# argumentcomputer/multi-stark

Hardware: AMD Instinct MI355X
Metric: prove_trace_rows_per_sec (higher is better)
Workload: dtype u64; 1 GPU; U32-add + byte-table lookup (benches/multi_stark.rs), 2^20 additions per proof, bench_config(): log_blowup 2, 100 queries, 10+10 PoW bits, GoldilocksBlake3Config; witness (traces + claims, 64-bit words) in pinned host memory at step start: upload, from_stage_1 on the device and read-back inside the timed region; the library narrows byte-valued traces on host threads INSIDE the step before they cro; rows_per_proof=1048832, proof_bytes=1100053, parallelism=single GPU

## Files before the change

multi-stark_amd/csrc/prover.hip:

```cpp
#include <algorithm>
#include <chrono>
#include <cstdio>
#include <cstdlib>

#include <sys/resource.h>
#include <unistd.h>

#include <atomic>
#include <condition_variable>
#include <functional>
#include <mutex>
#include <thread>

#include "host.h"
#include "ingest.h"
#include "lookup_params.h"
#include "open_plan.h"
#include "quotient_params.h"

namespace msamd {

namespace {
void load_block(const uint8_t* p, size_t len, u32 w[16]) {
  uint8_t buf[64];
  memset(buf, 0, 64);
  if (len) memcpy(buf, p, len);
  for (int i = 0; i < 16; i++)
    w[i] = (u32)buf[4 * i] | ((u32)buf[4 * i + 1] << 8) | ((u32)buf[4 * i + 2] << 16) | ((u32)buf[4 * i + 3] << 24);
}
void subtree_cv(const uint8_t* in, size_t len, u64 chunk_index, u32 root_flag, u32 out[8]) {
  if (len <= 1024) {
    b3_iv(out);
    size_t nblocks = len == 0 ? 1 : (len + 63) / 64;
    for (size_t b = 0; b < nblocks; b++) {
      size_t off = b * 64, bl = len - off < 64 ? len - off : 64;
      u32 m[16];
      load_block(in + off, bl, m);
      u32 flags = (b == 0 ? B3_CHUNK_START : 0) | (b == nblocks - 1 ? (B3_CHUNK_END | root_flag) : 0);
      b3_compress(out, m, chunk_index, (u32)bl, flags);
    }
    return;
  }
  size_t full = (len - 1) / 1024, lc = 1;
  while (lc * 2 <= full) lc *= 2;
  u32 m[16];
  subtree_cv(in, lc * 1024, chunk_index, 0, m);
  subtree_cv(in + lc * 1024, len - lc * 1024, chunk_index + lc, 0, m + 8);
  b3_iv(out);
  b3_compress(out, m, 0, 64, B3_PARENT | root_flag);
}
double now_ms() {
  return std::chrono::duration<double, std::milli>(std::chrono::steady_clock::now().time_since_epoch()).count();
}

struct HostProbes {
  bool on = false;
  double t0 = 0;
  long faults0 = 0;
  struct Mark {
    const char* what;
    double t;
    long faults;
  };
  std::vector<Mark> marks;
  static long faults_now() {
    struct rusage ru;
    return getrusage(RUSAGE_THREAD, &ru) == 0 ? ru.ru_minflt : 0;
  }
  void start() {
    on = getenv("MSAMD_TRACE_HOST") != nullptr;
    marks.clear();
    t0 = now_ms();
    if (on) faults0 = faults_now();
  }
  void mark(const char* what) {
    if (on) marks.push_back(Mark{what, now_ms(), faults_now()});
  }
  void print() const {
    if (!on) return;
    double prev = t0;
    long pf = faults0;
    for (auto& m : marks) {
      fprintf(stderr, "[msamd]   %-34s at %8.1f us (+%7.1f)  page faults +%ld\n", m.what, 1e3 * (m.t - t0), 1e3 * (m.t - prev), m.faults - pf);
      prev = m.t;
      pf = m.faults;
    }
  }
};
thread_local HostProbes g_probes;
}

void blake3_host(const uint8_t* in, size_t len, uint8_t out[32]) {
  u32 cv[8];
  subtree_cv(in, len, 0, B3_ROOT, cv);
  for (int i = 0; i < 8; i++)
    for (int k = 0; k < 4; k++) out[4 * i + k] = (uint8_t)(cv[i] >> (8 * k));
}

uint8_t Challenger::sample_byte() {
  if (output.empty()) {
    uint8_t d[32];
    blake3_host(input.data(), input.size(), d);
    input.assign(d, d + 32);
    output.assign(d, d + 32);
  }
  uint8_t b = output.back();
  output.pop_back();
  return b;
}
u64 Challenger::sample_u64() {
  u64 v = 0;
  for (int k = 0; k < 8; k++) v |= (u64)sample_byte() << (8 * k);
  return v;
}
u64 Challenger::sample_base() {
  for (;;) {
    u64 v = sample_u64();
    if (v < GL_P) return v;
  }
}
E2 Challenger::sample_ext() {
  u64 a = sample_base();
  u64 b = sample_base();
  return e2(a, b);
}
size_t Challenger::sample_bits(unsigned bits) { return (size_t)(sample_u64() & ((u64(1) << bits) - 1)); }

u64 Challenger::grind(unsigned bits) {
  if (bits == 0) return 0;
  std::vector<uint8_t> buf(input);
  size_t base = buf.size();
  buf.resize(base + 8);
  const u64 mask = (u64(1) << bits) - 1;
  for (u64 w = 0;; w++) {
    for (int k = 0; k < 8; k++) buf[base + k] = (uint8_t)(w >> (8 * k));
    uint8_t d[32];
    blake3_host(buf.data(), buf.size(), d);
    u64 v = 0;
    for (int k = 0; k < 8; k++) v |= (u64)d[31 - k] << (8 * k);
    if ((v & mask) == 0) {
      observe(w);
      size_t s = sample_bits(bits);
      if (s != 0) throw std::runtime_error("grind: internal inconsistency");
      return w;
    }
  }
}

namespace {
struct Reader {
  const uint8_t* p;
  size_t n, off = 0;
  u64 word() {
    if (off + 8 > n) throw std::runtime_error("system blob truncated");
    u64 v;
    memcpy(&v, p + off, 8);
    off += 8;
    return v;
  }
};
const u64 BLOB_MAGIC = 0x31305359534D0000ULL;
}

void commit_matrices(Ctx& ctx, std::vector<DMat>&& ldes, unsigned cap_height, PcsData& out) {
  out.ldes = std::move(ldes);
  out.tree = DTree();
  out.tree.cap_height = cap_height;
  for (auto& m : out.ldes) {
    out.tree.mat_d.push_back(m.d());
    out.tree.mat_h.push_back(m.h);
    out.tree.mat_w.push_back(m.w);
  }
  merkle_build(ctx, out.tree);
}

static DMat lde_of_host_matrix(Ctx& ctx, const u64* rowmajor_dev, size_t h, size_t w, unsigned lb) {
  unsigned logn = log2_strict(h);
  DBuf<u64> ev(ctx, h * w);
  transpose_in(ctx, rowmajor_dev, ev.p, h, w, true);
  DMat lde;
  lde.h = h << lb;
  lde.w = w;
  lde.buf = DBuf<u64>(ctx, lde.h * w);
  coset_lde(ctx, ev.p, lde.d(), logn, lb, w);
  return lde;
}

std::unique_ptr<HSystem> system_from_blob(Ctx& ctx, const uint8_t* blob, size_t len) {
  HIP_CHECK(hipSetDevice(ctx.device));
  Reader rd{blob, len};
  if (rd.word() != BLOB_MAGIC) throw std::runtime_error("bad system blob magic");
  std::unique_ptr<HSystem> sys(new HSystem());
  sys->ctx = &ctx;
  Params& p = sys->params;
  p.log_blowup = rd.word();
  p.cap_height = rd.word();
  p.log_final_poly_len = rd.word();
  p.max_log_arity = rd.word();
  p.num_queries = rd.word();
  p.commit_pow_bits = rd.word();
  p.query_pow_bits = rd.word();
  if (p.max_log_arity < 1 || p.max_log_arity > FRI_MAX_LOG_ARITY) throw std::runtime_error("max_log_arity must be 1 .. 6 (a FRI row is hashed as one BLAKE3 chunk)");
  if (p.log_blowup < 1 || p.log_blowup > 8) throw std::runtime_error("log_blowup out of range");
  if (p.commit_pow_bits > 40 || p.query_pow_bits > 40) throw std::runtime_error("proof-of-work bits out of range");
  {
    const char* tag = "multi-stark/v0";
    sys->seed.assign(tag, tag + 14);
    const u64 ps[7] = {p.log_blowup, p.cap_height, p.log_final_poly_len, p.max_log_arity, p.num_queries, p.commit_pow_bits,
                       p.query_pow_bits};
    for (u64 x : ps)
      for (int k = 0; k < 8; k++) sys->seed.push_back((uint8_t)(x >> (8 * k)));
  }
  const size_t D = 2;
  size_t nc = rd.word();
  std::vector<DMat> pre_ldes;
  for (size_t ci = 0; ci < nc; ci++) {
    sys->circuits.emplace_back();
    HCircuit& c = sys->circuits.back();
    c.main_width = rd.word();
    c.pre_width = rd.word();
    c.pre_height = rd.word();
    size_t nn = rd.word(), nz = rd.word(), nl = rd.word();
    c.num_lookups = nl;
    c.stage2_width = std::max<size_t>(nl, 1) * D;
    c.nodes.resize(nn);
    c.degrees.resize(nn);
    for (size_t i = 0; i < nn; i++) {
      u64 w0 = rd.word();
      PNode& nd = c.nodes[i];
      nd.kind = (uint32_t)(w0 & 0xff);
      nd.source = (uint32_t)((w0 >> 8) & 0xff);
      nd.offset = (uint32_t)((w0 >> 16) & 0xff);
// ... 216 lines not shown
void check_claims(size_t n_claims, const u64* offsets, const u64* data) {
  if (offsets[0] != 0) throw std::runtime_error("claim offsets must start at 0");
  for (size_t i = 0; i < n_claims; i++)
    if (offsets[i + 1] < offsets[i]) throw std::runtime_error("claim offsets must be non-decreasing");
  for (size_t i = 0, tot = (size_t)offsets[n_claims]; i < tot; i++)
    if (data[i] >= GL_P) throw std::runtime_error("non-canonical claim value");
}
}

std::unique_ptr<HWitness> witness_create_device(HSystem& sys, const ms_dev_matrix* traces, size_t n_claims, const u64* claim_offsets,
                                                const u64* claim_data, bool claims_on_device, void* producer_stream) {
  Ctx& ctx = *sys.ctx;
  HIP_CHECK(hipSetDevice(ctx.device));
  const size_t C = sys.circuits.size();
  if (!traces) throw std::runtime_error("ms_witness_create_device: null trace list");
  if (!claim_offsets) throw std::runtime_error("ms_witness_create_device: null claim offsets");
  std::vector<IngestView> views(C);
  std::vector<size_t> heights(C, 0);
  for (size_t ci = 0; ci < C; ci++) {
    const HCircuit& c = sys.circuits[ci];
    const size_t h = (size_t)traces[ci].height;
    heights[ci] = h;
    if (h == 0) continue;
    if (h & (h - 1)) throw std::runtime_error("trace height must be a power of two");
    if (log2_strict(h) > NTT_MAX_LOG || log2_strict(h) + sys.params.log_blowup > TW_LOG)
      throw std::runtime_error("trace height exceeds the supported maximum");
    if (c.pre_width && h != c.pre_height) throw std::runtime_error("main trace height must equal preprocessed trace height");
    views[ci] = ingest_check(ctx, traces[ci], ci, c.main_width, 8);
  }
  size_t tot = 0;
  if (claims_on_device) {
    ingest_check_device_range(ctx, claim_offsets, (n_claims + 1) * 8, 8, "device claim offsets");
  } else {
    tot = (size_t)claim_offsets[n_claims];
    if (tot && !claim_data) throw std::runtime_error("ms_witness_create_device: null claim data");
    check_claims(n_claims, claim_offsets, claim_data);
  }
  ingest_wait_for_producer(ctx, producer_stream);
  try {
    DBuf<u64> bad(ctx, C);
    if (C) HIP_CHECK(hipMemsetAsync(bad.p, 0xFF, C * 8, ctx.stream));
    std::vector<DBuf<u64>> dtr(C);
    for (size_t ci = 0; ci < C; ci++) {
      if (!heights[ci]) continue;
      dtr[ci] = DBuf<u64>(ctx, heights[ci] * views[ci].w);
      ingest_goldilocks(ctx, views[ci], dtr[ci].p, bad.p + ci);
    }
    DBuf<u64> d_offs(ctx, n_claims + 1), d_data;
    u64 tot_dev = 0;
    if (claims_on_device) {
      HIP_CHECK(hipMemcpyAsync(d_offs.p, claim_offsets, (n_claims + 1) * 8, hipMemcpyDeviceToDevice, ctx.stream));
      ctx.d2h_queue(&tot_dev, claim_offsets + n_claims, 8);
    } else {
      d_data = DBuf<u64>(ctx, std::max<size_t>(tot, 1));
      ctx.h2d(d_offs.p, claim_offsets, (n_claims + 1) * 8);
      if (tot) ctx.h2d(d_data.p, claim_data, tot * 8);
    }
    std::vector<u64> bad_h(C, ~u64(0));
    ctx.d2h(bad_h.data(), bad.p, C * 8);
    for (size_t ci = 0; ci < C; ci++)
      if (heights[ci] && bad_h[ci] != ~u64(0)) throw std::runtime_error(ingest_offender_text(ci, bad_h[ci], views[ci].w));
    if (claims_on_device) {
      if (tot_dev >> 60) throw std::runtime_error("device claims: the last offset is out of range");
      tot = (size_t)tot_dev;
      if (tot) {
        if (!claim_data) throw std::runtime_error("ms_witness_create_device: null claim data");
        ingest_check_device_range(ctx, claim_data, tot * 8, 8, "device claim data");
      }
      d_data = DBuf<u64>(ctx, std::max<size_t>(tot, 1));
      if (tot) HIP_CHECK(hipMemcpyAsync(d_data.p, claim_data, tot * 8, hipMemcpyDeviceToDevice, ctx.stream));
    }
    std::unique_ptr<HWitness> w = witness_from_device(sys, std::move(dtr), heights, std::move(d_offs), std::move(d_data), n_claims, tot);
    if (claims_on_device) check_claims(n_claims, w->claim_offsets.data(), w->claim_data.data());
    return w;
  } catch (...) {
    (void)hipStreamSynchronize(ctx.stream);
    abandon_pending();
    throw;
  }
}

std::unique_ptr<HWitness> witness_create(HSystem& sys, const u64* const* traces, const u64* heights, const u64* const* mult,
                                         const u64* const* args, size_t n_claims, const u64* claim_offsets, const u64* claim_data) {
  Ctx& ctx = *sys.ctx;
  HIP_CHECK(hipSetDevice(ctx.device));
  std::unique_ptr<HWitness> w(new HWitness());
  w->sys = &sys;
  size_t C = sys.circuits.size();
  w->traces.resize(C);
  w->lookups.resize(C);
  for (size_t ci = 0; ci < C; ci++) {
    const HCircuit& c = sys.circuits[ci];
    size_t h = heights[ci];
    w->heights.push_back(h);
    if (h == 0) continue;
    if (h & (h - 1)) throw std::runtime_error("trace height must be a power of two");
    if (log2_strict(h) > NTT_MAX_LOG || log2_strict(h) + sys.params.log_blowup > TW_LOG)
      throw std::runtime_error("trace height exceeds the supported maximum");
    if (c.pre_width && h != c.pre_height) throw std::runtime_error("main trace height must equal preprocessed trace height");
    if (!traces[ci]) {
      w->has_remote = true;
      continue;
    }
    size_t cnt = h * c.main_width;
    for (size_t i = 0; i < cnt; i++)
      if (traces[ci][i] >= GL_P) throw std::runtime_error("non-canonical trace value");
    w->traces[ci] = DBuf<u64>(ctx, cnt);
    ctx.h2d(w->traces[ci].p, traces[ci], cnt * 8);
    DLookups& lk = w->lookups[ci];
    lk.height = h;
    lk.num_lookups = c.num_lookups;
    lk.args_width = c.args_width;
    if (c.num_lookups == 0) continue;
    std::vector<uint32_t> offs(1, 0);
    for (auto& l : c.lookups) offs.push_back(offs.back() + (uint32_t)l.second.size());
    lk.arg_offsets = DBuf<uint32_t>(ctx, offs.size());
    ctx.h2d(lk.arg_offsets.p, offs.data(), offs.size() * 4);
    if (!(mult && mult[ci]) && c.stage2_trace_jit.function && !getenv("MSAMD_MATERIALISE_LOOKUPS") && !getenv("MSAMD_HOST_LOOKUP_VALUES")) continue;
    lk.mult = DBuf<u64>(ctx, h * c.num_lookups);
    lk.args = DBuf<u64>(ctx, std::max<size_t>(h * c.args_width, 1));
    if (mult && mult[ci]) {
      ctx.h2d(lk.mult.p, mult[ci], h * c.num_lookups * 8);
      if (c.args_width) ctx.h2d(lk.args.p, args[ci], h * c.args_width * 8);
      ctx.sync();
    } else if (c.prefix_on_device && !getenv("MSAMD_HOST_LOOKUP_VALUES") &&
               lookup_values_device(ctx, c.prefix_prog, w->traces[ci].p, c.pre_width ? c.d_preprocessed.p : nullptr, h, c.main_width,
                                    c.pre_width, c.args_width, lk.mult.p, lk.args.p)) {
      ctx.sync();
    } else {
      std::vector<u64> hm, ha;
      host_lookup_values(c, traces[ci], h, hm, ha);
      ctx.h2d(lk.mult.p, hm.data(), hm.size() * 8);
      if (!ha.empty()) ctx.h2d(lk.args.p, ha.data(), ha.size() * 8);
      ctx.sync();
    }
  }
  w->claim_offsets.assign(claim_offsets, claim_offsets + n_claims + 1);
  size_t tot = n_claims ? (size_t)claim_offsets[n_claims] : 0;
  if (claim_offsets[0] != 0) throw std::runtime_error("claim offsets must start at 0");
  for (size_t i = 0; i < n_claims; i++)
    if (claim_offsets[i + 1] < claim_offsets[i]) throw std::runtime_error("claim offsets must be non-decreasing");
  w->claim_data.assign(claim_data, claim_data + tot);
  w->claim_elems_total = tot;
  for (u64 x : w->claim_data)
    if (x >= GL_P) throw std::runtime_error("non-canonical claim value");
  w->d_claim_offsets = DBuf<u64>(ctx, n_claims + 1);
  w->d_claim_data = DBuf<u64>(ctx, std::max<size_t>(tot, 1));
  ctx.h2d(w->d_claim_offsets.p, w->claim_offsets.data(), (n_claims + 1) * 8);
  if (tot) ctx.h2d(w->d_claim_data.p, w->claim_data.data(), tot * 8);
  ctx.sync();
  return w;
}

u64 narrow_range(const u64* in, uint8_t* out, unsigned pb, size_t n);
namespace {
class PackPool {
 public:
  static PackPool* get(int device) {
    static std::mutex mu;
    static std::map<int, PackPool*> pools;
    static const int n_threads = []() {
      int n = 16;
      if (const char* e = getenv("MSAMD_PACK_THREADS")) n = atoi(e);
      return n > 64 ? 64 : n;
    }();
    if (n_threads <= 0) return nullptr;
    std::lock_guard<std::mutex> lk(mu);
    auto it = pools.find(device);
    if (it != pools.end()) return it->second;
    PackPool* p = new PackPool(n_threads);
    pools[device] = p;
    return p;
  }
  static constexpr size_t MAX_CHUNKS = 64, MAX_SUB = 128;
  size_t n_chunks = 0;
  void start(const u64* in, uint8_t* out, unsigned pb, size_t cnt, size_t chunks) {
    job_mu_.lock();
    std::unique_lock<std::mutex> lk(mu_);
    done_cv_.wait(lk, [&] { return busy_ == 0; });
    in_ = in, out_ = out, pb_ = pb, cnt_ = cnt;
    caller_ = std::this_thread::get_id();
    straggle_us_ = getenv("MSAMD_PACK_STRAGGLE_US") ? (unsigned)atoi(getenv("MSAMD_PACK_STRAGGLE_US")) : 0;
    n_chunks = std::max<size_t>(1, std::min(chunks, MAX_CHUNKS));
    per_chunk_ = ((cnt + n_chunks - 1) / n_chunks + 63) & ~size_t(63);
    n_chunks = (cnt + per_chunk_ - 1) / per_chunk_;
    next_.store(0);
    acc_.store(0);
    nsub_ = std::min<size_t>(2 * threads_.size(), MAX_SUB);
    for (size_t k = 0; k < n_chunks; k++) left_[k].store((int)nsub_);
    for (size_t i = 0; i < n_chunks * nsub_; i++) state_[i].store(0, std::memory_order_relaxed);
    busy_ = (int)threads_.size();
    gen_++;
    cv_.notify_all();
  }
  size_t chunk_begin(size_t k) const { return std::min(cnt_, k * per_chunk_); }
  bool wait_chunk(size_t k) {
    double all_claimed_at = 0;
    while (left_[k].load(std::memory_order_acquire) != 0) {
      if (next_.load(std::memory_order_relaxed) >= (k + 1) * nsub_) {
        const double now = now_ms();
        if (all_claimed_at == 0) all_claimed_at = now;
        if (now - all_claimed_at > 0.03) {
          for (size_t sub = 0; sub < nsub_ && left_[k].load(std::memory_order_acquire) != 0; sub++)
            if (state_[k * nsub_ + sub].load(std::memory_order_acquire) != 2) work_piece(k * nsub_ + sub, true);
          continue;
        }
      }
      if (!take_piece()) std::this_thread::yield();
    }
    return (acc_.load() >> (8 * pb_)) == 0;
  }
  void finish() { job_mu_.unlock(); }
  void quiesce() {
    std::unique_lock<std::mutex> lk(mu_);
    done_cv_.wait(lk, [&] { return busy_ == 0; });
  }
  struct Job {
    PackPool& p;
    Job(PackPool& pool, const u64* in, uint8_t* out, unsigned pb, size_t cnt, size_t chunks) : p(pool) { p.start(in, out, pb, cnt, chunks); }
    ~Job() { p.finish(); }
  };

 private:
  explicit PackPool(int n) {
    for (int i = 0; i < n; i++) threads_.emplace_back([this]() { run(); });
    for (auto& t : threads_) t.detach();
  }
  bool take_piece() {
    const size_t it = next_.fetch_add(1);
    if (it >= n_chunks * nsub_) return false;
    work_piece(it, false);
    return true;
  }
  void work_piece(size_t it, bool again) {
    const size_t k = it / nsub_, sub = it % nsub_;
    if (!again) {
      uint8_t unclaimed = 0;
      if (!state_[it].compare_exchange_strong(unclaimed, 1, std::memory_order_acq_rel)) return;
      if (straggle_us_ && sub == 3 && std::this_thread::get_id() != caller_)
        std::this_thread::sleep_for(std::chrono::microseconds(straggle_us_));
    }
    u64 acc = 0;
    const size_t b = chunk_begin(k), e = chunk_begin(k + 1);
    const size_t piece = (((e - b) + nsub_ - 1) / nsub_ + 7) & ~size_t(7);
    const size_t lo = std::min(e, b + sub * piece), hi = std::min(e, lo + piece);
    if (hi > lo) acc = narrow_range(in_ + lo, out_ + lo * pb_, pb_, hi - lo);
    if (acc) acc_.fetch_or(acc);
    if (state_[it].exchange(2, std::memory_order_acq_rel) != 2) left_[k].fetch_sub(1, std::memory_order_release);
  }
  void run() {
    uint64_t seen = 0;
    for (;;) {
      {
        std::unique_lock<std::mutex> lk(mu_);
        cv_.wait(lk, [&] { return gen_ != seen; });
        seen = gen_;
      }
      while (take_piece()) {
      }
      {
        std::unique_lock<std::mutex> lk(mu_);
        if (--busy_ == 0) done_cv_.notify_all();
      }
    }
  }
  std::vector<std::thread> threads_;
  std::mutex mu_, job_mu_;
  std::condition_variable cv_, done_cv_;
  uint64_t gen_ = 0;
  int busy_ = 0;
  const u64* in_ = nullptr;
  uint8_t* out_ = nullptr;
  unsigned pb_ = 1;
  size_t cnt_ = 0, per_chunk_ = 0, nsub_ = 1;
  std::atomic<uint8_t> state_[MAX_CHUNKS * MAX_SUB];
  std::thread::id caller_;
  unsigned straggle_us_ = 0;
  std::atomic<size_t> next_{0};
  std::atomic<u64> acc_{0};
  std::atomic<int> left_[MAX_CHUNKS];
};
}

void HWitness::pin(const void* p, size_t bytes) {
  if (!p || !bytes) return;
  const int r = host_range_pin(p, bytes);
  if (r == 1)
    registered.push_back(const_cast<void*>(p));
  else if (r == 0)
    pinned = false;
}
HWitness::~HWitness() {
  if (!host_resident) return;
  if (sys && sys->ctx) {
    (void)hipSetDevice(sys->ctx->device);
    (void)hipStreamSynchronize(sys->ctx->copy_stream);
    (void)hipStreamSynchronize(sys->ctx->claims_stream);
    if (sys->ctx->side_stream) (void)hipStreamSynchronize(sys->ctx->side_stream);
    (void)hipStreamSynchronize(sys->ctx->main_stream);
  }
  for (auto& st : stage)
    for (auto& e : st.ev)
      if (e) (void)hipEventDestroy(e);
  bool any_packed = false;
  for (uint8_t* p : h_packed) any_packed = any_packed || p != nullptr;
  if (any_packed)
    if (PackPool* pool = PackPool::get(sys && sys->ctx ? sys->ctx->device : 0)) pool->quiesce();
  for (void* p : registered) host_range_unpin(p);
  for (uint8_t* p : h_packed)
    if (p) (void)hipHostFree(p);
  (void)hipGetLastError();
}

std::unique_ptr<HWitness> witness_create_host(HSystem& sys, const u64* const* traces, const u64* heights, size_t n_claims,
                                              const u64* claim_offsets, const u64* claim_data, size_t data_first, size_t data_count,
                                              const u64* head, size_t n_head) {
  Ctx& ctx = *sys.ctx;
  HIP_CHECK(hipSetDevice(ctx.device));
  std::unique_ptr<HWitness> w(new HWitness());
  w->sys = &sys;
  w->host_resident = true;
  const size_t C = sys.circuits.size();
  w->traces.resize(C);
  w->lookups.resize(C);
  w->h_traces.assign(C, nullptr);
  w->h_mult.resize(C);
  w->h_args.resize(C);
  w->pack_bytes.assign(C, 0);
  w->h_packed.assign(C, nullptr);
  size_t pack_min = size_t(4) << 20;
  if (const char* e = getenv("MSAMD_PACK_MIN_BYTES")) pack_min = (size_t)atoll(e);
  const bool may_pack = !getenv("MSAMD_NO_PACK") && PackPool::get(ctx.device) != nullptr;
  for (size_t ci = 0; ci < C; ci++) {
    const HCircuit& c = sys.circuits[ci];
    const size_t h = heights[ci];
    w->heights.push_back(h);
    if (h == 0) continue;
    if (h & (h - 1)) throw std::runtime_error("trace height must be a power of two");
    if (log2_strict(h) > NTT_MAX_LOG || log2_strict(h) + sys.params.log_blowup > TW_LOG)
      throw std::runtime_error("trace height exceeds the supported maximum");
    if (c.pre_width && h != c.pre_height) throw std::runtime_error("main trace height must equal preprocessed trace height");
    if (!traces[ci]) {
      w->has_remote = true;
      continue;
    }
    const size_t cnt = h * c.main_width;
    u64 seen = 0;
    for (size_t i = 0; i < cnt; i++) {
      if (traces[ci][i] >= GL_P) throw std::runtime_error("non-canonical trace value");
      seen |= traces[ci][i];
    }
    w->h_traces[ci] = traces[ci];
    w->pin(traces[ci], cnt * 8);
    if (may_pack && cnt * 8 >= pack_min && (seen >> 32) == 0) {
      const unsigned pb = (seen >> 8) == 0 ? 1 : (seen >> 16) == 0 ? 2 : 4;
      void* hp = nullptr;
      if (hipHostMalloc(&hp, cnt * pb, hipHostMallocDefault) == hipSuccess) {
        w->pack_bytes[ci] = pb;
        w->h_packed[ci] = (uint8_t*)hp;
      } else {
        (void)hipGetLastError();
      }
    }
    DLookups& lk = w->lookups[ci];
    lk.height = h;
    lk.num_lookups = c.num_lookups;
    lk.args_width = c.args_width;
    if (c.num_lookups == 0) continue;
    std::vector<uint32_t> offs(1, 0);
    for (auto& l : c.lookups) offs.push_back(offs.back() + (uint32_t)l.second.size());
    lk.arg_offsets = DBuf<uint32_t>(ctx, offs.size());
    ctx.h2d(lk.arg_offsets.p, offs.data(), offs.size() * 4);
    unsigned threads = 64;
    const bool fits = c.prefix_on_device && c.prefix_prog.n_slots * threads * 8 <= 64 * 1024 && !getenv("MSAMD_HOST_LOOKUP_VALUES");
    if (!fits) {
      host_lookup_values(c, traces[ci], h, w->h_mult[ci], w->h_args[ci]);
      w->pin(w->h_mult[ci].data(), w->h_mult[ci].size() * 8);
      w->pin(w->h_args[ci].data(), w->h_args[ci].size() * 8);
    }
  }
  if (claim_offsets[0] != 0) throw std::runtime_error("claim offsets must start at 0");
  for (size_t i = 0; i < n_claims; i++)
    if (claim_offsets[i + 1] < claim_offsets[i]) throw std::runtime_error("claim offsets must be non-decreasing");
  const size_t tot = n_claims ? (size_t)claim_offsets[n_claims] : 0;
  w->claim_offsets.assign(claim_offsets, claim_offsets + n_claims + 1);
  w->claim_elems_total = tot;
  if (data_count == ~size_t(0)) {
    w->claim_data.assign(claim_data, claim_data + tot);
  } else {
    if (data_first > tot || data_count > tot - data_first) throw std::runtime_error("claims slice outside the claims' data");
    const size_t need_head = std::min<size_t>(tot, 130);
    if (n_head < need_head || (need_head && !head)) throw std::runtime_error("claims slice: the first 130 elements are needed on every rank");
    w->claims_partial = true;
    w->has_remote = true;
    w->claim_elem0 = data_first;
    w->claim_data.assign(claim_data, claim_data + data_count);
    w->claim_head.assign(head, head + need_head);
    for (u64 x : w->claim_head)
      if (x >= GL_P) throw std::runtime_error("non-canonical claim value");
  }
  for (u64 x : w->claim_data)
    if (x >= GL_P) throw std::runtime_error("non-canonical claim value");
  w->pin(w->claim_offsets.data(), (n_claims + 1) * 8);
  w->pin(w->claim_data.data(), w->claim_data.size() * 8);
  ctx.sync();
  return w;
}

namespace {
struct HostUpload {
  HWitness& w;
  Ctx& ctx;
  bool on = false;
  bool skip_claims = false;
  HostUpload(HWitness& wit, Ctx& c) : w(wit), ctx(c) {}
  bool fused(size_t ci) const {
    const HCircuit& c = w.sys->circuits[ci];
    return w.host_resident && c.stage2_trace_jit.function && w.h_mult[ci].empty();
  }
  void issue(HWitness::Staged& st) {
    HSystem& sys = *w.sys;
    const size_t C = sys.circuits.size();
    for (auto& e : st.ev)
      if (!e) HIP_CHECK(hipEventCreateWithFlags(&e, hipEventDisableTiming));
    st.clear();
    st.traces.resize(C);
    st.mult.resize(C);
    st.args.resize(C);
    HIP_CHECK(hipEventRecord(ctx.copy_ev[3], ctx.stream));
    HIP_CHECK(hipStreamWaitEvent(ctx.copy_stream, ctx.copy_ev[3], 0));
    ctx.side_config();
    ctx.copy_delay();
    HIP_CHECK(hipStreamWaitEvent(ctx.claims_stream, ctx.copy_ev[3], 0));
    const size_t n_claims = w.claim_offsets.size() - 1, tot = w.claim_data.size();
    auto from_caller = [&](void* dst, const void* src, size_t bytes, hipStream_t s) {
      if (w.pinned)
        HIP_CHECK(hipMemcpyAsync(dst, src, bytes, hipMemcpyHostToDevice, s));
      else
        ctx.bounce_h2d(dst, src, bytes, s);
    };
    for (size_t ci = 0; ci < C; ci++) {
      const HCircuit& c = sys.circuits[ci];
      const size_t h = w.heights[ci];
      if (!h || !w.h_traces[ci]) continue;
      const size_t cnt = h * c.main_width;
      st.traces[ci] = DBuf<u64>(ctx, cnt);
      const unsigned pb = w.pack_bytes[ci];
      PackPool* pool = pb && !w.prefetch ? PackPool::get(ctx.device) : nullptr;
      bool sent = false;
      if (pool) {
        static const size_t n_chunks = getenv("MSAMD_PACK_CHUNKS") ? (size_t)atoi(getenv("MSAMD_PACK_CHUNKS")) : 8;
        PackPool::Job job(*pool, w.h_traces[ci], w.h_packed[ci], pb, cnt, n_chunks);
        sent = true;
        for (size_t k = 0; k < pool->n_chunks; k++) {
          if (!pool->wait_chunk(k)) {
            sent = false;
            break;
          }
          if (k == 0) g_probes.mark("narrow upload: first chunk ready");
          const size_t b = pool->chunk_begin(k), e = pool->chunk_begin(k + 1);
          pull_widen_words(w.h_packed[ci] + b * pb, pb, e - b, st.traces[ci].p + b, ctx.copy_stream);
        }
        g_probes.mark("narrow upload: last chunk queued");
      }
      if (!sent) from_caller(st.traces[ci].p, w.h_traces[ci], cnt * 8, ctx.copy_stream);
    }
    HIP_CHECK(hipEventRecord(st.ev[0], ctx.copy_stream));
    st.has_host_lookups = false;
    for (size_t ci = 0; ci < C; ci++) {
      const HCircuit& c = sys.circuits[ci];
      const size_t h = w.heights[ci];
      if (!h || !c.num_lookups || !w.h_traces[ci]) continue;
      if (fused(ci)) continue;
      st.mult[ci] = DBuf<u64>(ctx, h * c.num_lookups);
      st.args[ci] = DBuf<u64>(ctx, std::max<size_t>(h * c.args_width, 1));
      if (!w.h_mult[ci].empty()) {
        st.has_host_lookups = true;
        from_caller(st.mult[ci].p, w.h_mult[ci].data(), w.h_mult[ci].size() * 8, ctx.copy_stream);
        if (!w.h_args[ci].empty()) from_caller(st.args[ci].p, w.h_args[ci].data(), w.h_args[ci].size() * 8, ctx.copy_stream);
      }
    }
    if (!skip_claims) {
      st.claim_offsets = DBuf<u64>(ctx, n_claims + 1);
      st.claim_data = DBuf<u64>(ctx, std::max<size_t>(tot, 1));
      from_caller(st.claim_offsets.p, w.claim_offsets.data(), (n_claims + 1) * 8, ctx.copy_stream);
      if (tot) from_caller(st.claim_data.p, w.claim_data.data(), tot * 8, ctx.copy_stream);
    }
    HIP_CHECK(hipEventRecord(st.ev[2], ctx.copy_stream));
    for (size_t ci = 0; ci < C; ci++) {
      const HCircuit& c = sys.circuits[ci];
      const size_t h = w.heights[ci];
      if (!h || !c.num_lookups || !w.h_mult[ci].empty() || fused(ci) || !w.h_traces[ci]) continue;
      if (!lookup_values_device(ctx, c.prefix_prog, st.traces[ci].p, c.pre_width ? c.d_preprocessed.p : nullptr, h, c.main_width, c.pre_width,
                                c.args_width, st.mult[ci].p, st.args[ci].p, ctx.copy_stream))
        throw std::runtime_error("host-resident witness: lookup prefix does not fit the device sweep");
    }
    HIP_CHECK(hipEventRecord(st.ev[1], ctx.copy_stream));
    st.valid = true;
  }
  void start() {
    if (!w.host_resident) return;
    on = true;
    if (w.prefetch && w.stage[w.cur ^ 1].valid)
      w.cur ^= 1;
    else
      issue(w.stage[w.cur]);
    HWitness::Staged& st = w.stage[w.cur];
    for (size_t ci = 0; ci < st.traces.size(); ci++) {
      w.traces[ci] = std::move(st.traces[ci]);
      w.lookups[ci].mult = std::move(st.mult[ci]);
      w.lookups[ci].args = std::move(st.args[ci]);
    }
    w.d_claim_offsets = std::move(st.claim_offsets);
    w.d_claim_data = std::move(st.claim_data);
    st.valid = false;
    if (w.prefetch) issue(w.stage[w.cur ^ 1]);
  }
  void wait_traces() {
    if (on) HIP_CHECK(hipStreamWaitEvent(ctx.stream, w.stage[w.cur].ev[0], 0));
  }
  void lookup_values() {
    if (!on) return;
    HIP_CHECK(hipStreamWaitEvent(ctx.stream, w.stage[w.cur].ev[1], 0));
    if (ctx.side_forked && ctx.stream != ctx.side_stream) HIP_CHECK(hipStreamWaitEvent(ctx.side_stream, w.stage[w.cur].ev[1], 0));
  }
  void wait_claims() {
    if (on) HIP_CHECK(hipStreamWaitEvent(ctx.stream, w.stage[w.cur].ev[2], 0));
  }
  ~HostUpload() {
    if (!on) return;
    (void)hipStreamSynchronize(ctx.copy_stream);
    (void)hipStreamSynchronize(ctx.claims_stream);
    for (auto& t : w.traces) t.reset();
    for (auto& lk : w.lookups) {
      lk.mult.reset();
      lk.args.reset();
    }
    w.d_claim_offsets.reset();
    w.d_claim_data.reset();
  }
};
}

namespace {
struct PW {
  std::vector<uint8_t> b;
  void u8(uint8_t x) { b.push_back(x); }
  void u64_(u64 x) {
    size_t o = b.size();
    b.resize(o + 8);
    memcpy(&b[o], &x, 8);
  }
  void ext(E2 e) {
    u64_(e.c0);
    u64_(e.c1);
  }
  void raw(const void* p, size_t n) {
    const uint8_t* q = (const uint8_t*)p;
    b.insert(b.end(), q, q + n);
  }
  void cap(const std::vector<Digest>& c) {
    u64_(c.size());
    for (auto& d : c) raw(d.b, 32);
  }
};
typedef std::vector<std::vector<std::vector<E2>>> OpenedRound;
void write_round(PW& w, const OpenedRound& r) {
  w.u64_(r.size());
  for (auto& m : r) {
    w.u64_(m.size());
    for (auto& pt : m) {
      w.u64_(pt.size());
      for (auto& e : pt) w.ext(e);
    }
  }
}

struct OpenRound {
  PcsData* data;
  std::vector<std::vector<E2>> points;
};

struct SymbolicPoints {
  const E2* d_points = nullptr;
  size_t n = 0;
  std::function<void(std::vector<E2>& values)> resolve;
  std::vector<int> next_log;
};

struct PhaseTrace {
  Ctx& ctx;
  bool on;
  double t;
  explicit PhaseTrace(Ctx& c) : ctx(c), on(getenv("MSAMD_TRACE") != nullptr), t(0) {
    if (on) {
      ctx.sync();
      t = now_ms();
    }
  }
  void mark(const char* what) {
    if (!on) return;
    ctx.sync();
    double n = now_ms();
    fprintf(stderr, "[msamd] %-22s %8.3f ms\n", what, n - t);
    t = n;
  }
};

u64 grind(Ctx& ctx, Challenger& ch, unsigned bits) {
  if (bits == 0) return 0;
  u64 w = 0;
  if (bits >= 4 && grind_device(ctx, ch.input, bits, &w)) {
    ch.observe(w);
    if (ch.sample_bits(bits) != 0) throw std::runtime_error("grind: device witness rejected by the host challenger");
    return w;
  }
// ... 1177 lines not shown
```

Before: 158.0 million rows/s.

## Send trace tail wide on a second stream while host narrowing is still in progress

The pack pool moves into a header and gains a two-ended cursor. While the caller waits for narrowed chunks and the copy links are idle, it takes groups of pieces from the end of the trace and uploads them unnarrowed (8-byte words) on the claims stream, so the PCIe link stays busy instead of idling until the CPU narrowing finishes. This trades more bytes over the link for less waiting on host packing. It adds event polling and a cross-stream wait before later work consumes the trace.

```diff
diff --git a/multi-stark_amd/csrc/pack_pool.h b/multi-stark_amd/csrc/pack_pool.h
--- /dev/null
+++ b/multi-stark_amd/csrc/pack_pool.h
@@ -0,0 +1,221 @@
+#pragma once
+#include <algorithm>
+#include <atomic>
+#include <chrono>
+#include <condition_variable>
+#include <cstddef>
+#include <cstdint>
+#include <cstdlib>
+#include <functional>
+#include <map>
+#include <mutex>
+#include <thread>
+#include <vector>
+
+namespace msamd {
+
+uint64_t narrow_range(const uint64_t* in, uint8_t* out, unsigned pb, size_t n);
+
+struct WideLink {
+  std::function<bool()> idle;
+  std::function<void(size_t begin, size_t end)> send;
+  size_t group_elems = (size_t(1) << 20) / 8;
+};
+
+class PackPool {
+ public:
+  static PackPool* get(int device) {
+    static std::mutex mu;
+    static std::map<int, PackPool*> pools;
+    static const int n_threads = []() {
+      int n = 16;
+      if (const char* e = getenv("MSAMD_PACK_THREADS")) n = atoi(e);
+      return n > 64 ? 64 : n;
+    }();
+    if (n_threads <= 0) return nullptr;
+    std::lock_guard<std::mutex> lk(mu);
+    auto it = pools.find(device);
+    if (it != pools.end()) return it->second;
+    PackPool* p = new PackPool(n_threads);
+    pools[device] = p;
+    return p;
+  }
+  static PackPool* create(int n_threads) { return new PackPool(n_threads); }
+
+  static constexpr size_t MAX_CHUNKS = 64, MAX_SUB = 128;
+  size_t n_chunks = 0;
+  double redo_after_ms = 0.03;
+  void start(const uint64_t* in, uint8_t* out, unsigned pb, size_t cnt, size_t chunks, const WideLink* wide = nullptr) {
+    job_mu_.lock();
+    std::unique_lock<std::mutex> lk(mu_);
+    done_cv_.wait(lk, [&] { return busy_ == 0; });
+    in_ = in, out_ = out, pb_ = pb, cnt_ = cnt;
+    caller_ = std::this_thread::get_id();
+    straggle_us_ = getenv("MSAMD_PACK_STRAGGLE_US") ? (unsigned)atoi(getenv("MSAMD_PACK_STRAGGLE_US")) : 0;
+    slow_us_ = getenv("MSAMD_PACK_SLOW_US") ? (unsigned)atoi(getenv("MSAMD_PACK_SLOW_US")) : 0;
+    n_chunks = std::max<size_t>(1, std::min(chunks, MAX_CHUNKS));
+    per_chunk_ = ((cnt + n_chunks - 1) / n_chunks + 63) & ~size_t(63);
+    n_chunks = (cnt + per_chunk_ - 1) / per_chunk_;
+    acc_.store(0);
+    nsub_ = std::min<size_t>(2 * threads_.size(), MAX_SUB);
+    const size_t pieces = n_chunks * nsub_;
+    cursor_.store(uint64_t(pieces) << 32);
+    for (size_t k = 0; k < n_chunks; k++) left_[k].store((int)nsub_);
+    for (size_t i = 0; i < pieces; i++) state_[i].store(0, std::memory_order_relaxed);
+    wide_ = wide && wide->idle && wide->send ? wide : nullptr;
+    wide_elems_ = 0, groups_ = 0;
+    group_pieces_ = 1;
+    if (wide_ && pieces) {
+      const size_t piece = piece_elems(0);
+      group_pieces_ = std::max<size_t>(1, (wide_->group_elems + piece - 1) / std::max<size_t>(piece, 1));
+    }
+    busy_ = (int)threads_.size();
+    gen_++;
+    cv_.notify_all();
+  }
+  size_t chunk_begin(size_t k) const { return std::min(cnt_, k * per_chunk_); }
+  size_t narrow_end(size_t k) const {
+    const size_t border = piece_begin(size_t(cursor_.load(std::memory_order_acquire) >> 32));
+    return std::min(chunk_begin(k + 1), std::max(chunk_begin(k), border));
+  }
+  size_t wide_elems() const { return wide_elems_; }
+  size_t wide_groups() const { return groups_; }
+  bool wait_chunk(size_t k) {
+    double all_claimed_at = 0;
+    while (left_[k].load(std::memory_order_acquire) != 0) {
+      if (wide_ && take_group()) continue;
+      const uint64_t c = cursor_.load(std::memory_order_relaxed);
+      if ((c & 0xffffffffu) >= std::min<uint64_t>((k + 1) * nsub_, c >> 32)) {
+        const double now = now_ms();
+        if (all_claimed_at == 0) all_claimed_at = now;
+        if (now - all_claimed_at > redo_after_ms) {
+          for (size_t sub = 0; sub < nsub_ && left_[k].load(std::memory_order_acquire) != 0; sub++)
+            if (state_[k * nsub_ + sub].load(std::memory_order_acquire) != 2) work_piece(k * nsub_ + sub, true);
+          continue;
+        }
+      }
+      if (!take_piece()) std::this_thread::yield();
+    }
+    return (acc_.load() >> (8 * pb_)) == 0;
+  }
+  void finish() {
+    wide_ = nullptr;
+    job_mu_.unlock();
+  }
+  void quiesce() {
+    std::unique_lock<std::mutex> lk(mu_);
+    done_cv_.wait(lk, [&] { return busy_ == 0; });
+  }
+  struct Job {
+    PackPool& p;
+    Job(PackPool& pool, const uint64_t* in, uint8_t* out, unsigned pb, size_t cnt, size_t chunks, const WideLink* wide = nullptr) : p(pool) {
+      p.start(in, out, pb, cnt, chunks, wide);
+    }
+    ~Job() { p.finish(); }
+  };
+
+ private:
+  static double now_ms() {
+    return std::chrono::duration<double, std::milli>(std::chrono::steady_clock::now().time_since_epoch()).count();
+  }
+  explicit PackPool(int n) {
+    for (int i = 0; i < n; i++) threads_.emplace_back([this]() { run(); });
+    for (auto& t : threads_) t.detach();
+  }
+  size_t piece_elems(size_t k) const {
+    const size_t b = chunk_begin(k), e = chunk_begin(k + 1);
+    return (((e - b) + nsub_ - 1) / nsub_ + 7) & ~size_t(7);
+  }
+  size_t piece_begin(size_t it) const {
+    if (it >= n_chunks * nsub_) return cnt_;
+    const size_t k = it / nsub_, sub = it % nsub_;
+    return std::min(chunk_begin(k + 1), chunk_begin(k) + sub * piece_elems(k));
+  }
+  bool take_piece() {
+    uint64_t c = cursor_.load(std::memory_order_relaxed);
+    for (;;) {
+      if ((c & 0xffffffffu) >= (c >> 32)) return false;
+      if (cursor_.compare_exchange_weak(c, c + 1, std::memory_order_acq_rel, std::memory_order_relaxed)) break;
+    }
+    work_piece(size_t(c & 0xffffffffu), false);
+    return true;
+  }
+  bool take_group() {
+    uint64_t c = cursor_.load(std::memory_order_relaxed);
+    if ((c >> 32) - (c & 0xffffffffu) <= group_pieces_) return false;
+    if (!wide_->idle()) return false;
+    size_t first, end;
+    for (;;) {
+      const uint64_t next = c & 0xffffffffu;
+      end = size_t(c >> 32);
+      if (end - next <= group_pieces_) return false;
+      first = end - group_pieces_;
+      if (cursor_.compare_exchange_weak(c, (uint64_t(first) << 32) | next, std::memory_order_acq_rel, std::memory_order_relaxed)) break;
+    }
+    const size_t b = piece_begin(first), e = piece_begin(end);
+    for (size_t it = first; it < end; it++) {
+      state_[it].store(2, std::memory_order_release);
+      left_[it / nsub_].fetch_sub(1, std::memory_order_release);
+    }
+    if (e > b) {
+      wide_->send(b, e);
+      wide_elems_ += e - b;
+      groups_++;
+    }
+    return true;
+  }
+  void work_piece(size_t it, bool again) {
+    const size_t k = it / nsub_, sub = it % nsub_;
+    if (!again) {
+      uint8_t unclaimed = 0;
+      if (!state_[it].compare_exchange_strong(unclaimed, 1, std::memory_order_acq_rel)) return;
+      if (straggle_us_ && sub == 3 && std::this_thread::get_id() != caller_)
+        std::this_thread::sleep_for(std::chrono::microseconds(straggle_us_));
+    }
+    uint64_t acc = 0;
+    const size_t lo = piece_begin(it), hi = std::min(chunk_begin(k + 1), lo + piece_elems(k));
+    if (hi > lo) acc = narrow_range(in_ + lo, out_ + lo * pb_, pb_, hi - lo);
+    if (acc) acc_.fetch_or(acc);
+    if (state_[it].exchange(2, std::memory_order_acq_rel) != 2) left_[k].fetch_sub(1, std::memory_order_release);
+  }
+  void run() {
+    uint64_t seen = 0;
+    for (;;) {
+      unsigned slow_us;
+      {
+        std::unique_lock<std::mutex> lk(mu_);
+        cv_.wait(lk, [&] { return gen_ != seen; });
+        seen = gen_;
+        slow_us = slow_us_;
+      }
+      for (;;) {
+        if (slow_us) std::this_thread::sleep_for(std::chrono::microseconds(slow_us));
+        if (!take_piece()) break;
+      }
+      {
+        std::unique_lock<std::mutex> lk(mu_);
+        if (--busy_ == 0) done_cv_.notify_all();
+      }
+    }
+  }
+  std::vector<std::thread> threads_;
+  std::mutex mu_, job_mu_;
+  std::condition_variable cv_, done_cv_;
+  uint64_t gen_ = 0;
+  int busy_ = 0;
+  const uint64_t* in_ = nullptr;
+  uint8_t* out_ = nullptr;
+  unsigned pb_ = 1;
+  size_t cnt_ = 0, per_chunk_ = 0, nsub_ = 1;
+  std::atomic<uint8_t> state_[MAX_CHUNKS * MAX_SUB];
+  std::thread::id caller_;
+  unsigned straggle_us_ = 0;
+  unsigned slow_us_ = 0;
+  const WideLink* wide_ = nullptr;
+  size_t group_pieces_ = 1, wide_elems_ = 0, groups_ = 0;
+  std::atomic<uint64_t> cursor_{0};
+  std::atomic<uint64_t> acc_{0};
+  std::atomic<int> left_[MAX_CHUNKS];
+};
+
+}
diff --git a/multi-stark_amd/csrc/prover.hip b/multi-stark_amd/csrc/prover.hip
--- a/multi-stark_amd/csrc/prover.hip
+++ b/multi-stark_amd/csrc/prover.hip
@@ -16,6 +16,7 @@
 #include "ingest.h"
 #include "lookup_params.h"
 #include "open_plan.h"
+#include "pack_pool.h"
 #include "quotient_params.h"
 
 namespace msamd {
@@ -63,6 +64,10 @@
     long faults;
   };
   std::vector<Mark> marks;
+  struct Upload {
+    size_t circuit, narrow_bytes, wide_bytes, groups;
+  };
+  std::vector<Upload> uploads;
   static long faults_now() {
     struct rusage ru;
     return getrusage(RUSAGE_THREAD, &ru) == 0 ? ru.ru_minflt : 0;
@@ -70,14 +75,21 @@
   void start() {
     on = getenv("MSAMD_TRACE_HOST") != nullptr;
     marks.clear();
+    uploads.clear();
     t0 = now_ms();
     if (on) faults0 = faults_now();
   }
   void mark(const char* what) {
     if (on) marks.push_back(Mark{what, now_ms(), faults_now()});
   }
+  void upload(size_t circuit, size_t narrow_bytes, size_t wide_bytes, size_t groups) {
+    if (on) uploads.push_back(Upload{circuit, narrow_bytes, wide_bytes, groups});
+  }
   void print() const {
     if (!on) return;
+    for (auto& u : uploads)
+      fprintf(stderr, "[msamd]   narrow upload: trace %zu: %zu bytes sent narrow, %zu bytes sent wide in %zu groups\n", u.circuit, u.narrow_bytes,
+              u.wide_bytes, u.groups);
     double prev = t0;
     long pf = faults0;
     for (auto& m : marks) {
@@ -600,135 +612,6 @@
   return w;
 }
 
-u64 narrow_range(const u64* in, uint8_t* out, unsigned pb, size_t n);
-namespace {
-class PackPool {
- public:
-  static PackPool* get(int device) {
-    static std::mutex mu;
-    static std::map<int, PackPool*> pools;
-    static const int n_threads = []() {
-      int n = 16;
-      if (const char* e = getenv("MSAMD_PACK_THREADS")) n = atoi(e);
-      return n > 64 ? 64 : n;
-    }();
-    if (n_threads <= 0) return nullptr;
-    std::lock_guard<std::mutex> lk(mu);
-    auto it = pools.find(device);
-    if (it != pools.end()) return it->second;
-    PackPool* p = new PackPool(n_threads);
-    pools[device] = p;
-    return p;
-  }
-  static constexpr size_t MAX_CHUNKS = 64, MAX_SUB = 128;
-  size_t n_chunks = 0;
-  void start(const u64* in, uint8_t* out, unsigned pb, size_t cnt, size_t chunks) {
-    job_mu_.lock();
-    std::unique_lock<std::mutex> lk(mu_);
-    done_cv_.wait(lk, [&] { return busy_ == 0; });
-    in_ = in, out_ = out, pb_ = pb, cnt_ = cnt;
-    caller_ = std::this_thread::get_id();
-    straggle_us_ = getenv("MSAMD_PACK_STRAGGLE_US") ? (unsigned)atoi(getenv("MSAMD_PACK_STRAGGLE_US")) : 0;
-    n_chunks = std::max<size_t>(1, std::min(chunks, MAX_CHUNKS));
-    per_chunk_ = ((cnt + n_chunks - 1) / n_chunks + 63) & ~size_t(63);
-    n_chunks = (cnt + per_chunk_ - 1) / per_chunk_;
-    next_.store(0);
-    acc_.store(0);
-    nsub_ = std::min<size_t>(2 * threads_.size(), MAX_SUB);
-    for (size_t k = 0; k < n_chunks; k++) left_[k].store((int)nsub_);
-    for (size_t i = 0; i < n_chunks * nsub_; i++) state_[i].store(0, std::memory_order_relaxed);
-    busy_ = (int)threads_.size();
-    gen_++;
-    cv_.notify_all();
-  }
-  size_t chunk_begin(size_t k) const { return std::min(cnt_, k * per_chunk_); }
-  bool wait_chunk(size_t k) {
-    double all_claimed_at = 0;
-    while (left_[k].load(std::memory_order_acquire) != 0) {
-      if (next_.load(std::memory_order_relaxed) >= (k + 1) * nsub_) {
-        const double now = now_ms();
-        if (all_claimed_at == 0) all_claimed_at = now;
-        if (now - all_claimed_at > 0.03) {
-          for (size_t sub = 0; sub < nsub_ && left_[k].load(std::memory_order_acquire) != 0; sub++)
-            if (state_[k * nsub_ + sub].load(std::memory_order_acquire) != 2) work_piece(k * nsub_ + sub, true);
-          continue;
-        }
-      }
-      if (!take_piece()) std::this_thread::yield();
-    }
-    return (acc_.load() >> (8 * pb_)) == 0;
-  }
-  void finish() { job_mu_.unlock(); }
-  void quiesce() {
-    std::unique_lock<std::mutex> lk(mu_);
-    done_cv_.wait(lk, [&] { return busy_ == 0; });
-  }
-  struct Job {
-    PackPool& p;
-    Job(PackPool& pool, const u64* in, uint8_t* out, unsigned pb, size_t cnt, size_t chunks) : p(pool) { p.start(in, out, pb, cnt, chunks); }
-    ~Job() { p.finish(); }
-  };
-
- private:
-  explicit PackPool(int n) {
-    for (int i = 0; i < n; i++) threads_.emplace_back([this]() { run(); });
-    for (auto& t : threads_) t.detach();
-  }
-  bool take_piece() {
-    const size_t it = next_.fetch_add(1);
-    if (it >= n_chunks * nsub_) return false;
-    work_piece(it, false);
-    return true;
-  }
-  void work_piece(size_t it, bool again) {
-    const size_t k = it / nsub_, sub = it % nsub_;
-    if (!again) {
-      uint8_t unclaimed = 0;
-      if (!state_[it].compare_exchange_strong(unclaimed, 1, std::memory_order_acq_rel)) return;
-      if (straggle_us_ && sub == 3 && std::this_thread::get_id() != caller_)
-        std::this_thread::sleep_for(std::chrono::microseconds(straggle_us_));
-    }
-    u64 acc = 0;
-    const size_t b = chunk_begin(k), e = chunk_begin(k + 1);
-    const size_t piece = (((e - b) + nsub_ - 1) / nsub_ + 7) & ~size_t(7);
-    const size_t lo = std::min(e, b + sub * piece), hi = std::min(e, lo + piece);
-    if (hi > lo) acc = narrow_range(in_ + lo, out_ + lo * pb_, pb_, hi - lo);
-    if (acc) acc_.fetch_or(acc);
-    if (state_[it].exchange(2, std::memory_order_acq_rel) != 2) left_[k].fetch_sub(1, std::memory_order_release);
-  }
-  void run() {
-    uint64_t seen = 0;
-    for (;;) {
-      {
-        std::unique_lock<std::mutex> lk(mu_);
-        cv_.wait(lk, [&] { return gen_ != seen; });
-        seen = gen_;
-      }
-      while (take_piece()) {
-      }
-      {
-        std::unique_lock<std::mutex> lk(mu_);
-        if (--busy_ == 0) done_cv_.notify_all();
-      }
-    }
-  }
-  std::vector<std::thread> threads_;
-  std::mutex mu_, job_mu_;
-  std::condition_variable cv_, done_cv_;
-  uint64_t gen_ = 0;
-  int busy_ = 0;
-  const u64* in_ = nullptr;
-  uint8_t* out_ = nullptr;
-  unsigned pb_ = 1;
-  size_t cnt_ = 0, per_chunk_ = 0, nsub_ = 1;
-  std::atomic<uint8_t> state_[MAX_CHUNKS * MAX_SUB];
-  std::thread::id caller_;
-  unsigned straggle_us_ = 0;
-  std::atomic<size_t> next_{0};
-  std::atomic<u64> acc_{0};
-  std::atomic<int> left_[MAX_CHUNKS];
-};
-}
 
 void HWitness::pin(const void* p, size_t bytes) {
   if (!p || !bytes) return;
@@ -898,18 +781,54 @@
       bool sent = false;
       if (pool) {
         static const size_t n_chunks = getenv("MSAMD_PACK_CHUNKS") ? (size_t)atoi(getenv("MSAMD_PACK_CHUNKS")) : 8;
-        PackPool::Job job(*pool, w.h_traces[ci], w.h_packed[ci], pb, cnt, n_chunks);
-        sent = true;
-        for (size_t k = 0; k < pool->n_chunks; k++) {
-          if (!pool->wait_chunk(k)) {
-            sent = false;
-            break;
+        bool pulls_pending = false, wide_pending = false;
+        WideLink link;
+        link.idle = [&]() {
+          for (int i = 1; i <= 2; i++) {
+            bool& pending = i == 1 ? pulls_pending : wide_pending;
+            if (!pending) continue;
+            const hipError_t r = hipEventQuery(ctx.copy_ev[i]);
+            if (r == hipErrorNotReady) {
+              (void)hipGetLastError();
+              return false;
+            }
+            HIP_CHECK(r);
+            pending = false;
           }
-          if (k == 0) g_probes.mark("narrow upload: first chunk ready");
-          const size_t b = pool->chunk_begin(k), e = pool->chunk_begin(k + 1);
-          pull_widen_words(w.h_packed[ci] + b * pb, pb, e - b, st.traces[ci].p + b, ctx.copy_stream);
+          return true;
+        };
+        link.send = [&](size_t b, size_t e) {
+          from_caller(st.traces[ci].p + b, w.h_traces[ci] + b, (e - b) * 8, ctx.claims_stream);
+          HIP_CHECK(hipEventRecord(ctx.copy_ev[2], ctx.claims_stream));
+          wide_pending = true;
+        };
+        const bool wide_tail = w.pinned && !getenv("MSAMD_NO_WIDE_TAIL");
+        size_t groups = 0, wide_words = 0;
+        {
+          PackPool::Job job(*pool, w.h_traces[ci], w.h_packed[ci], pb, cnt, n_chunks, wide_tail ? &link : nullptr);
+          sent = true;
+          for (size_t k = 0; k < pool->n_chunks; k++) {
+            if (!pool->wait_chunk(k)) {
+              sent = false;
+              break;
+            }
+            if (k == 0) g_probes.mark("narrow upload: first chunk ready");
+            const size_t b = pool->chunk_begin(k), e = pool->narrow_end(k);
+            if (e == b) continue;
+            pull_widen_words(w.h_packed[ci] + b * pb, pb, e - b, st.traces[ci].p + b, ctx.copy_stream);
+            if (wide_tail) {
+              HIP_CHECK(hipEventRecord(ctx.copy_ev[1], ctx.copy_stream));
+              pulls_pending = true;
+            }
+          }
+          groups = pool->wide_groups(), wide_words = pool->wide_elems();
         }
         g_probes.mark("narrow upload: last chunk queued");
+        if (groups) {
+          HIP_CHECK(hipEventRecord(ctx.copy_ev[2], ctx.claims_stream));
+          HIP_CHECK(hipStreamWaitEvent(ctx.copy_stream, ctx.copy_ev[2], 0));
+        }
+        g_probes.upload(ci, sent ? (cnt - wide_words) * 8 : 0, sent ? wide_words * 8 : cnt * 8, groups);
       }
       if (!sent) from_caller(st.traces[ci].p, w.h_traces[ci], cnt * 8, ctx.copy_stream);
     }
```

New measurement: 153.3 million rows/s. 3.0% lower.
